# AbrahamSanders/realtime-codec-agent

Measured on AMD Instinct MI355X. Metric: batch-encode audio-hours/hour (+ xRT and p50 frame-step latency of 1 duplex stream in `duplex`), higher is better.
Workload: dtype f32; 1 GPU; batch MagiCodec-style encode, 16 kHz stereo, 0.1 s chunks / 2.0 s context, 256 windows per step (BASELINE configs[1]); codebook=131072x16

## Files before the change

realtime_codec_agent_amd/csrc/rca_codec.hip:

```cpp
#include <stdarg.h>

#include <algorithm>
#include <array>
#include <cmath>
#include <map>
#include <type_traits>

#include "rca_common.h"

namespace rca {
thread_local char g_err[512] = {0};
}
using namespace rca;

typedef float f32x16 __attribute__((ext_vector_type(16)));

#define RCA_LAT_MAX_FRAMES 64
#define RCA_LDS_BUDGET (152 * 1024)

typedef float f32x4 __attribute__((ext_vector_type(4)));

struct RowSrc {
    const float* base;
    int C;
    long chan_stride;
    long win_stride;
    int T;
    const long* row_off = nullptr;
    long span = 0;
    __device__ __forceinline__ long off(long b) const {
        return row_off ? row_off[b] : (b % C) * chan_stride + (b / C) * win_stride;
    }
};

__device__ __forceinline__ float lrelu(float v, float slope) { return v >= 0.0f ? v : v * slope; }

template <int KS>
__global__ __launch_bounds__(256) void conv_in_kernel(RowSrc src, const float* __restrict__ w,
                                                      const float* __restrict__ bias, float* __restrict__ y,
                                                      int B, int Cout, int Lout) {
    const long idx = (long)blockIdx.x * blockDim.x + threadIdx.x;
    if (idx >= (long)B * Lout) return;
    const int b = (int)(idx / Lout);
    const int t = (int)(idx - (long)b * Lout);
    const float* xr = src.base + src.off(b);
    constexpr int padL = KS / 2;
    float xv[KS];
#pragma unroll
    for (int kk = 0; kk < KS; ++kk) {
        const int i = t + kk - padL;
        xv[kk] = (i >= 0 && i < src.T) ? xr[i] : 0.0f;
    }
    float* yo = y + (long)b * Cout * Lout + t;
    for (int co = 0; co < Cout; ++co) {
        float acc = bias[co];
#pragma unroll
        for (int kk = 0; kk < KS; ++kk) {
            const int i = t + kk - padL;
            if (i >= 0 && i < src.T) acc = __builtin_fmaf(w[co * KS + kk], xv[kk], acc);
        }
        yo[(long)co * Lout] = acc;
    }
}

__global__ __launch_bounds__(256) void conv1d_chain_kernel(const float* __restrict__ x, const float* __restrict__ w,
                                                           const float* __restrict__ bias, float* __restrict__ y,
                                                           int B, int Cin, int Lin, int Cout, int Lout, int k, int s,
                                                           int pre, float slope, int clamp_out) {
    const long idx = (long)blockIdx.x * blockDim.x + threadIdx.x;
    if (idx >= (long)B * Cout * Lout) return;
    const int t = (int)(idx % Lout);
    const long r = idx / Lout;
    const int co = (int)(r % Cout);
    const int b = (int)(r / Cout);
    const int padL = (k - s + 1) / 2;
    const float* xb = x + (long)b * Cin * Lin;
    const float* wr = w + (long)co * Cin * k;
    float acc = bias[co];
    const int i0 = t * s - padL;
    for (int ci = 0; ci < Cin; ++ci) {
        const float* xr = xb + (long)ci * Lin;
        for (int kk = 0; kk < k; ++kk) {
            const int i = i0 + kk;
            if (i >= 0 && i < Lin) {
                float v = xr[i];
                if (pre) v = lrelu(v, slope);
                acc = __builtin_fmaf(wr[ci * k + kk], v, acc);
            }
        }
    }
    if (clamp_out) acc = acc > 1.0f ? 1.0f : (acc < -1.0f ? -1.0f : acc);
    y[idx] = acc;
}

__global__ __launch_bounds__(256) void convtr1d_chain_kernel(const float* __restrict__ x, const float* __restrict__ w,
                                                             const float* __restrict__ bias, float* __restrict__ y,
                                                             int B, int Cin, int Lin, int Cout, int k, int s, int pre,
                                                             float slope) {
    const int Lout = Lin * s;
    const long idx = (long)blockIdx.x * blockDim.x + threadIdx.x;
    if (idx >= (long)B * Cout * Lout) return;
    const int u = (int)(idx % Lout);
    const long r = idx / Lout;
    const int co = (int)(r % Cout);
    const int b = (int)(r / Cout);
    const int padL = (k - s + 1) / 2;
    const int kk0 = (u + padL) % s;
    const float* xb = x + (long)b * Cin * Lin;
    float acc = bias[co];
    for (int ci = 0; ci < Cin; ++ci) {
        const float* xr = xb + (long)ci * Lin;
        const float* wr = w + ((long)ci * Cout + co) * k;
        for (int kk = kk0; kk < k; kk += s) {
            const int t = (u + padL - kk) / s;
            if (t >= 0 && t < Lin) {
                float v = xr[t];
                if (pre) v = lrelu(v, slope);
                acc = __builtin_fmaf(wr[kk], v, acc);
            }
        }
    }
    y[idx] = acc;
}

typedef int rca_rsrc_t __attribute__((ext_vector_type(4)));
typedef float rca_f32x2_t __attribute__((ext_vector_type(2)));
__device__ float rca_buffer_load_f32(rca_rsrc_t rsrc, int voffset, int soffset, int aux) __asm("llvm.amdgcn.raw.buffer.load.f32");
__device__ rca_f32x2_t rca_buffer_load_f32x2(rca_rsrc_t rsrc, int voffset, int soffset, int aux) __asm("llvm.amdgcn.raw.buffer.load.v2f32");
typedef float rca_f32x4_t __attribute__((ext_vector_type(4)));
__device__ rca_f32x4_t rca_buffer_load_f32x4(rca_rsrc_t rsrc, int voffset, int soffset, int aux) __asm("llvm.amdgcn.raw.buffer.load.v4f32");
__device__ __forceinline__ rca_rsrc_t rca_make_rsrc(const void* base, int num_records) {
    const unsigned long a = (unsigned long)base;
    rca_rsrc_t r;
    r[0] = __builtin_amdgcn_readfirstlane((int)(unsigned)a);
    r[1] = __builtin_amdgcn_readfirstlane((int)((a >> 32) & 0xFFFF));
    r[2] = num_records;
    r[3] = 0x00020000;
    return r;
}

#ifdef RCA_CONV_TIMELINE
__device__ long* rca_prof_buf = nullptr;
#define RCA_TL_STAMP(v) const long v = tl_buf ? (long)wall_clock64() : 0
#define RCA_TL_ADD(acc, a, b) acc += (b) - (a)
#define RCA_TL_MIN(acc, a, b) acc = ((b) - (a)) < acc ? ((b) - (a)) : acc
#else
#define RCA_TL_STAMP(v)
#define RCA_TL_ADD(acc, a, b)
#define RCA_TL_MIN(acc, a, b)
#endif
template <int S>
struct ConvLds {
    static constexpr int want = (S == 8) ? 4 : (S == 4) ? 8 : (S == 2) ? 16 : (S == 5) ? 6 : 2;
    static constexpr int stride(int NT) {
        int u = NT + 2;
        while ((u % 32) != want % 32) ++u;
        return u;
    }
};

struct FuseIn {
    RowSrc src;
    const float* w_in;
    const float* b_in;
};
struct TrInfo {
    int s, padL, Lout, n_co;
};
template <int KS, int S, int TR>
struct ConvBOff {
    static constexpr int padL = (KS - S + 1) / 2;
    static constexpr int q_of(int kp, int half) {
        const int kl = 2 * kp + half, kk = kl % KS;
        const int d = TR ? -kk : kk - padL;
        return (d >= 0) ? d / S : -((-d + S - 1) / S);
    }
    static constexpr int off(int kp, int half, int U) {
        const int kl = 2 * kp + half, ci = kl / KS, kk = kl % KS;
        const int d = TR ? -kk : kk - padL;
        const int q = q_of(kp, half);
        return (ci * S + (d - q * S)) * U + 1 + q;
    }
    static constexpr int delta(int kp, int U) { return off(kp, 1, U) - off(kp, 0, U); }
    static constexpr int distinct(int k, int KPC, int U) {
        int found[4] = {0, 0, 0, 0};
        int n = 0;
        for (int kp = 0; kp < KPC; ++kp) {
            const int d = delta(kp, U);
            bool seen = false;
            for (int i = 0; i < n; ++i) seen = seen || found[i] == d;
            if (!seen && n < 4) found[n++] = d;
        }
        return found[k < n ? k : n - 1];
    }
    static constexpr int count(int KPC, int U) {
        int found[8] = {0, 0, 0, 0, 0, 0, 0, 0};
        int n = 0;
        for (int kp = 0; kp < KPC; ++kp) {
            const int d = delta(kp, U);
            bool seen = false;
            for (int i = 0; i < n; ++i) seen = seen || found[i] == d;
            if (!seen && n < 8) found[n++] = d;
        }
        return n;
    }
};

#ifndef RCA_CONV_WPB
#define RCA_CONV_WPB 1
#endif
#ifndef RCA_CONV_OCC
#define RCA_CONV_OCC 2
#endif
#ifndef RCA_CONV_PIPE
#define RCA_CONV_PIPE 1
#endif
#ifndef RCA_CONV_PRIO
#define RCA_CONV_PRIO 1
#endif
#ifndef RCA_CONV_ABUF
#define RCA_CONV_ABUF 1
#endif
#ifndef RCA_CONV_EPRIO
#define RCA_CONV_EPRIO 1
#endif
#ifdef RCA_ABL_NOBREAD
#define RCA_ABL_BREAD(x) (slope)
#else
#define RCA_ABL_BREAD(x) (x)
#endif
typedef __bf16 conv_bf16x8 __attribute__((ext_vector_type(8)));
typedef __bf16 conv_bf16x2 __attribute__((ext_vector_type(2)));
__device__ __forceinline__ unsigned conv_pack_bf16x2(float a, float b) {
    const conv_bf16x2 v = {(__bf16)a, (__bf16)b};
    return __builtin_bit_cast(unsigned, v);
}
template <int BF>
__device__ __forceinline__ void conv_split8(const float (&w)[8], uint4& hi, uint4& lo) {
    unsigned ph[4], pl[4];
#pragma unroll
    for (int j = 0; j < 4; ++j) {
        ph[j] = conv_pack_bf16x2(w[2 * j], w[2 * j + 1]);
        pl[j] = BF == 3 ? conv_pack_bf16x2(w[2 * j] - __uint_as_float(ph[j] << 16), w[2 * j + 1] - __uint_as_float(ph[j] & 0xffff0000u)) : 0u;
    }
    hi = make_uint4(ph[0], ph[1], ph[2], ph[3]);
    lo = make_uint4(pl[0], pl[1], pl[2], pl[3]);
}
template <int KS, int S, int CIC, int WM, int WN, int FUSE, int TR, int BF = 0, int FULLC = 0>
__global__ __launch_bounds__(64 * RCA_CONV_WPB, (((KS == 8 && CIC == 2) || (KS == 16 && CIC == 1)) && WM * WN < 8) ? 3 : RCA_CONV_OCC) void conv1d_mfma_kernel(const float* __restrict__ x, const float* __restrict__ wp,
                                                          const float* __restrict__ bias, float* __restrict__ y,
                                                          int Cin, int Lin, int Cout, int Lout, long Ncols, int nchunks,
                                                          int pre, float slope, FuseIn fin, TrInfo tr) {
    constexpr int MT = WM * 32;
    constexpr int NW = WN * 32;
    constexpr int U = ConvLds<S>::stride(NW);
    constexpr int KPC = CIC * KS / 2;
    constexpr int QPC = KPC / 4;
    constexpr int E = (NW + 2) * S;
    constexpr int PW = (S % 2 == 0 && !TR) ? 2 : 1;
    constexpr int RE = (E + 64 * PW - 1) / (64 * PW);
    constexpr int padL = (KS - S + 1) / 2;
    constexpr int BUF = CIC * S * U + 4;
    static_assert((CIC * KS) % 8 == 0, "chunk must hold whole weight quads");

    extern __shared__ __attribute__((aligned(16))) float xs_all[];
#ifdef RCA_CONV_TIMELINE
    long* const tl_buf = rca_prof_buf;
#endif
    RCA_TL_STAMP(tl0);

    const int lane = threadIdx.x & 63;
    const int half = lane >> 5;
    const int wave = __builtin_amdgcn_readfirstlane(threadIdx.x >> 6);
    float* xs = xs_all + wave * 2 * BUF;
    const int n_co_real = (Cout + MT - 1) / MT;
    const int n_co = TR ? n_co_real * tr.s : n_co_real;
    const long wg = blockIdx.x;
    const int xcd = (int)(wg & 7);
    const long seq = wg >> 3;
    const int co_tile_x = __builtin_amdgcn_readfirstlane((int)(seq % n_co));
    const int phase = TR ? co_tile_x / n_co_real : 0;
    const int co_tile = TR ? co_tile_x % n_co_real : co_tile_x;
    const long col_tile = (seq / n_co) * 8 + xcd;
// ... 296 lines not shown
#pragma unroll
            for (int wn = 0; wn < WN; ++wn) {
                float bv[8];
#pragma unroll
                for (int i = 0; i < 8; ++i) {
                    const int kp = g * 8 + i;
                    bv[i] = kp < KPC ? xb[b_off(kp < KPC ? kp : 0) + wn * 32] : 0.0f;
                    if (EDGE && kp < KPC && ((zmask[wn] >> kp) & 1u)) bv[i] = 0.0f;
                }
                conv_split8<BF>(bv, bh[wn], bl[wn]);
            }
#pragma unroll
            for (int wm = 0; wm < WM; ++wm) {
                float aw[8];
#pragma unroll
                for (int qq = 0; qq < 2; ++qq) {
                    const int q = 2 * g + qq;
                    const float4 q4 = q < QPC ? a[wm][q < QPC ? q : 0] : make_float4(0.0f, 0.0f, 0.0f, 0.0f);
                    aw[4 * qq + 0] = q4.x; aw[4 * qq + 1] = q4.y; aw[4 * qq + 2] = q4.z; aw[4 * qq + 3] = q4.w;
                }
                uint4 ah, al;
                conv_split8<BF>(aw, ah, al);
                const conv_bf16x8 ahv = __builtin_bit_cast(conv_bf16x8, ah), alv = __builtin_bit_cast(conv_bf16x8, al);
#pragma unroll
                for (int wn = 0; wn < WN; ++wn) {
                    const conv_bf16x8 bhv = __builtin_bit_cast(conv_bf16x8, bh[wn]);
                    acc[wm][wn] = __builtin_amdgcn_mfma_f32_32x32x16_bf16(ahv, bhv, acc[wm][wn], 0, 0, 0);
                    if (BF == 3) {
                        acc[wm][wn] = __builtin_amdgcn_mfma_f32_32x32x16_bf16(ahv, __builtin_bit_cast(conv_bf16x8, bl[wn]), acc[wm][wn], 0, 0, 0);
                        acc[wm][wn] = __builtin_amdgcn_mfma_f32_32x32x16_bf16(alv, bhv, acc[wm][wn], 0, 0, 0);
                    }
                }
#pragma unroll
                for (int qq = 0; qq < 2; ++qq) {
                    const int q = 2 * g + qq;
                    if (q < QPC) a[wm][q] = w_load(wm, cn, q);
                }
            }
        }
    };

    if (FUSE) stage_load(0);
    stage_write(0);
    __builtin_amdgcn_wave_barrier();
    if constexpr (PIPE) read_head(0);
    RCA_TL_STAMP(tl1);
#ifdef RCA_CONV_TIMELINE
    long tl_load = 1 << 30, tl_mfma = 0, tl_write = 0;
#endif
    const int lastc = nchunks - 1;
    auto chunk_loop = [&](auto edge_tag, auto act_tag) __attribute__((always_inline)) {
    for (int c = 0; c < nchunks; c += 2) {
        const int c1 = min(c + 1, lastc);
        RCA_TL_STAMP(ta);
        stage_load(c1);
        __builtin_amdgcn_sched_barrier(0);
        RCA_TL_STAMP(tb);
        __builtin_amdgcn_s_setprio(RCA_CONV_EPRIO);
        if constexpr (BF != 0) compute_b(0, c1, edge_tag);
        else if constexpr (PIPE) compute_p(0, c1, edge_tag);
        else compute_t(0, c1, edge_tag);
        __builtin_amdgcn_s_setprio(RCA_CONV_PRIO ? 3 : 2);
        __builtin_amdgcn_sched_barrier(0);
        RCA_TL_STAMP(tc);
        stage_write_t(1, act_tag);
        __builtin_amdgcn_wave_barrier();
        if constexpr (PIPE) {
            read_head(1);
            __builtin_amdgcn_sched_barrier(0);
        }
        RCA_TL_STAMP(td);
        RCA_TL_MIN(tl_load, tb, tc); RCA_TL_ADD(tl_mfma, tb, tc); RCA_TL_ADD(tl_write, tc, td);
        if (c + 1 >= nchunks) break;
        const int c2 = min(c + 2, lastc);
        stage_load(c2);
        __builtin_amdgcn_sched_barrier(0);
        __builtin_amdgcn_s_setprio(RCA_CONV_EPRIO);
        if constexpr (BF != 0) compute_b(1, c2, edge_tag);
        else if constexpr (PIPE) compute_p(1, c2, edge_tag);
        else compute_t(1, c2, edge_tag);
        __builtin_amdgcn_s_setprio(RCA_CONV_PRIO ? 3 : 2);
        __builtin_amdgcn_sched_barrier(0);
        stage_write_t(0, act_tag);
        __builtin_amdgcn_wave_barrier();
        if constexpr (PIPE) {
            read_head(0);
            __builtin_amdgcn_sched_barrier(0);
        }
    }
    };
    if (pre & 1) {
        if (edges) chunk_loop(std::true_type{}, std::true_type{});
        else chunk_loop(std::false_type{}, std::true_type{});
    } else {
        if (edges) chunk_loop(std::true_type{}, std::false_type{});
        else chunk_loop(std::false_type{}, std::false_type{});
    }

    if (RCA_CONV_EPRIO) __builtin_amdgcn_s_setprio(0);
    RCA_TL_STAMP(tl2);
    const long orow = TR ? tr.Lout : Lout;
    const bool full_rows = co0 + MT <= Cout;
    float* const yw = y + ((long)b_base * Cout + co0) * orow;
#pragma unroll
    for (int wn = 0; wn < WN; ++wn) {
        const int dn = 1 - lead + wn * 32 + (lane & 31);
        if (dn >= ncol_left) continue;
        int bb, t;
        rel_bt(dn, bb, t);
        int ocol = t;
        if (TR) {
            ocol = tr.s * t - tr.padL + phase;
            if (ocol < 0 || ocol >= (int)orow) continue;
        }
        const unsigned voff = ((unsigned)bb * (unsigned)(Cout * (int)orow) + (unsigned)ocol + (unsigned)(4 * half) * (unsigned)orow) * 4u;
        if (pre & 2) {
#pragma unroll
            for (int wm = 0; wm < WM; ++wm)
#pragma unroll
                for (int r = 0; r < 16; ++r) acc[wm][wn][r] = fmaxf(acc[wm][wn][r], acc[wm][wn][r] * slope);
        }
        if (full_rows) {
#pragma unroll
            for (int wm = 0; wm < WM; ++wm)
#pragma unroll
                for (int r = 0; r < 16; ++r) {
                    const int cu = wm * 32 + (r & 3) + 8 * (r >> 2);
                    char* const yr = reinterpret_cast<char*>(yw + (long)cu * orow);
                    *reinterpret_cast<float*>(yr + voff) = acc[wm][wn][r];
                }
        } else {
#pragma unroll
            for (int wm = 0; wm < WM; ++wm)
#pragma unroll
                for (int r = 0; r < 16; ++r) {
                    const int cu = wm * 32 + (r & 3) + 8 * (r >> 2);
                    char* const yr = reinterpret_cast<char*>(yw + (long)cu * orow);
                    if (co0 + cu + 4 * half < Cout) *reinterpret_cast<float*>(yr + voff) = acc[wm][wn][r];
                }
        }
    }
#ifdef RCA_CONV_TIMELINE
    if (tl_buf && lane == 0) {
        const long tl3 = (long)wall_clock64();
        const unsigned hw = __builtin_amdgcn_s_getreg((31 << 11) | (0 << 6) | 4);
        const unsigned xcc = __builtin_amdgcn_s_getreg((3 << 11) | (0 << 6) | 20);
        constexpr int region = KS == 4 ? 0 : KS == 8 ? 1 : KS == 10 ? 2 : KS == 16 ? 3 : KS == 3 ? 4 : 5;
        long* o = tl_buf + ((long)region * 65536 + ((blockIdx.x * RCA_CONV_WPB + wave) & 0xFFFF)) * 8;
        o[6] = tl_load | (tl_mfma << 32);
        o[7] = tl_write | ((long)nchunks << 32);
        o[0] = tl0; o[1] = tl1; o[2] = tl2; o[3] = tl3;
        o[4] = (long)hw | ((long)xcc << 32);
        o[5] = (long)KS | ((long)S << 8) | ((long)WM << 16) | ((long)wave << 24) | ((long)blockIdx.x << 32);
    }
#endif
}

template <int KS, int S, int CIC, int FUSE>
__global__ __launch_bounds__(512) void conv1d_ws_kernel(const float* __restrict__ x, const float* __restrict__ wp,
                                                        const float* __restrict__ bias, float* __restrict__ y,
                                                        int Cin, int Lin, int Cout, int Lout, long Ncols, int nchunks,
                                                        int pre, float slope, FuseIn fin) {
    constexpr int WM = 2, WN = 2;
    constexpr int MT = WM * 32, NW = WN * 32;
    constexpr int U = ConvLds<S>::stride(NW);
    constexpr int KPC = CIC * KS / 2;
    constexpr int QPC = KPC / 4;
    constexpr int E = (NW + 2) * S;
    constexpr int RE = (E + 63) / 64;
    constexpr int padL = (KS - S + 1) / 2;
    constexpr int BUF = CIC * S * U + 4;
    constexpr int WBUF = WM * QPC * 64 * 4;
    static_assert(KPC % 4 == 0 && KPC <= 64, "chunk shape");

    extern __shared__ __attribute__((aligned(16))) float lds[];
    float* aw_all = lds;
    float* xs_all = lds + 2 * WBUF;

    const int lane = threadIdx.x & 63;
    const int half = lane >> 5;
    const int wave = __builtin_amdgcn_readfirstlane(threadIdx.x >> 6);
    const bool producer = wave >= 4;
    const int cw = wave & 3;
    float* xs = xs_all + cw * 2 * BUF;

    const int n_co = (Cout + MT - 1) / MT;
    const long wg = blockIdx.x;
    const int xcd = (int)(wg & 7);
    const long seq = wg >> 3;
    const int co_tile = (int)(seq % n_co);
    const long col_tile = (seq / n_co) * 8 + xcd;
    const long n0 = (col_tile * 4 + cw) * NW;
    const int co0 = co_tile * MT;
    const bool active = n0 < Ncols;
    const long kquads = (long)nchunks * QPC;
    const int lastc = nchunks - 1;

    if (producer) {
        unsigned s_goff[RE];
        int s_loff[RE];
        bool s_ok[RE];
#pragma unroll
        for (int r = 0; r < RE; ++r) {
            const int e = lane + 64 * r;
            const int slot = e / S, p = e - slot * S;
            const long n = n0 - 1 + slot;
            s_ok[r] = active && e < E && n >= 0 && n < Ncols;
        s_loff[r] = e < E ? p * U + slot : -1;
            const long nn = s_ok[r] ? n : 0;
            const long b = nn / Lout;
            const int t = (int)(nn - b * Lout);
            s_goff[r] = s_ok[r] ? (unsigned)(b * Cin * (long)Lin + (long)t * S + p) : 0u;
        }
        float pc[FUSE ? RE : 1][7];
        if (FUSE) {
#pragma unroll
            for (int r = 0; r < RE; ++r) {
                const int e = lane + 64 * r;
                const int slot = e / S, p = e - slot * S;
                const long n = n0 - 1 + slot;
                const long nn = s_ok[r] ? n : 0;
                const long b = nn / Lout;
                const int i = (int)(nn - b * Lout) * S + p;
                const float* row = fin.src.base + fin.src.off(b);
#pragma unroll
                for (int kk = 0; kk < 7; ++kk) {
                    const int j = i + kk - 3;
                    pc[r][kk] = (s_ok[r] && j >= 0 && j < fin.src.T) ? row[j] : 0.0f;
                }
            }
        }
        const float act_slope = pre ? slope : 1.0f;
        constexpr int WITEMS = WM * QPC * 64;
        constexpr int WPER = (WITEMS + 255) / 256;
        const int ptid = threadIdx.x - 256;
        float sreg[CIC][RE];
        float4 wreg[WPER];
        auto issue_loads = [&](int c) {
#pragma unroll
            for (int i = 0; i < WPER; ++i) {
                const int it = ptid + 256 * i;
                const int itc = it < WITEMS ? it : 0;
                const int wm = itc / (QPC * 64), rem = itc - wm * (QPC * 64);
                const int cot = co_tile * WM + wm;
                wreg[i] = reinterpret_cast<const float4*>(wp)[((long)cot * kquads + (long)c * QPC) * 64 + rem];
            }
#pragma unroll
            for (int cl = 0; cl < CIC; ++cl) {
                const int ci = c * CIC + cl;
                if (FUSE) {
                    const int cc = ci < Cin ? ci : 0;
                    const float* wr = fin.w_in + cc * 7;
                    const float bi = fin.b_in[cc];
#pragma unroll
                    for (int r = 0; r < RE; ++r) {
                        float a = bi;
#pragma unroll
                        for (int kk = 0; kk < 7; ++kk) a = __builtin_fmaf(wr[kk], pc[r][kk], a);
                        sreg[cl][r] = a;
                    }
                } else {
                    const float* xc = x + (long)(ci < Cin ? ci : 0) * Lin;
#pragma unroll
                    for (int r = 0; r < RE; ++r) sreg[cl][r] = xc[s_goff[r]];
                }
            }
        };
        auto write_lds = [&](int c, int buf) {
            float4* aw = reinterpret_cast<float4*>(aw_all + buf * WBUF);
#pragma unroll
            for (int i = 0; i < WPER; ++i) {
                const int it = ptid + 256 * i;
                if (it < WITEMS) aw[it] = wreg[i];
            }
            float* dst = xs + buf * BUF;
#pragma unroll
            for (int cl = 0; cl < CIC; ++cl) {
                const bool cok = (c * CIC + cl) < Cin;
#pragma unroll
                for (int r = 0; r < RE; ++r) {
                    float v = (s_ok[r] && cok) ? sreg[cl][r] : 0.0f;
                    v = fmaxf(v, v * act_slope);
                    dst[s_loff[r] >= 0 ? cl * S * U + s_loff[r] : CIC * S * U] = v;
                }
            }
        };
        issue_loads(0);
        write_lds(0, 0);
        issue_loads(min(1, lastc));
        __syncthreads();
        for (int c = 0; c < nchunks; ++c) {
            const int c1 = min(c + 1, lastc);
            write_lds(c1, (c + 1) & 1);
            issue_loads(min(c + 2, lastc));
            __syncthreads();
        }
        return;
    }

    __builtin_amdgcn_s_setprio(3);
    int b_off[KPC];
    unsigned long long m_first = 0, m_last = 0;
#pragma unroll
    for (int kp = 0; kp < KPC; ++kp) {
        const int kl = 2 * kp + half;
        const int ci = kl / KS, kk = kl - ci * KS;
// ... 1084 lines not shown
    rca_codec* h = new rca_codec();
    h->cfg = *cfg;
    h->device = device;
    int rc = RCA_OK;
    auto bail = [&](int code) { rca_codec_destroy(h); return code; };
    if (hipStreamCreateWithFlags(&h->stream, hipStreamNonBlocking) != hipSuccess) return bail(fail(RCA_ERR_HIP, "stream create"));
    const int n = cfg->n_stages;
    h->hop = 1;
    for (int i = 0; i < n; ++i) h->hop *= cfg->strides[i];
    codec_receptive_field(*cfg, h->hop, &h->enc_left_frames, &h->dec_left_frames);

    auto add = [&](std::vector<ConvLayer>& v, const std::string& name, int cin, int cout, int k, int s, int pre, int tr,
                   bool pack) -> int {
        ConvLayer L;
        L.cin = cin; L.cout = cout; L.k = k; L.s = s; L.pre = pre; L.tr = tr;
        if ((rc = upload(ts, nt, name + ".weight", (long)cin * cout * k, &L.w)) != RCA_OK) return rc;
        if ((rc = upload(ts, nt, name + ".bias", cout, &L.b)) != RCA_OK) { v.push_back(L); return rc; }
        {
            const size_t nb = ((size_t)cout + 127) / 128 * 128 + 64;
            if (hipMalloc((void**)&L.bp, nb * 4) != hipSuccess || hipMemset(L.bp, 0, nb * 4) != hipSuccess ||
                hipMemcpy(L.bp, L.b, (size_t)cout * 4, hipMemcpyDeviceToDevice) != hipSuccess) {
                v.push_back(L);
                return fail(RCA_ERR_HIP, "bias pad alloc");
            }
        }
        if (pack && !tr && mfma_supported(k, s)) {
            const rca_tensor_t* t = find_tensor(ts, nt, name + ".weight");
            if ((rc = pack_weights((const float*)t->data, L)) != RCA_OK) { v.push_back(L); return rc; }
        }
        if (tr && k == 2 * s) {
            const rca_tensor_t* t = find_tensor(ts, nt, name + ".weight");
            if ((rc = pack_weights_tr((const float*)t->data, L)) != RCA_OK) { v.push_back(L); return rc; }
        }
        v.push_back(L);
        return RCA_OK;
    };
    if ((rc = add(h->enc, "enc.conv_in", 1, cfg->channels[0], cfg->k_in, 1, 0, 0, false)) != RCA_OK) return bail(rc);
    for (int i = 0; i < n; ++i) {
        const int s = cfg->strides[i];
        if ((rc = add(h->enc, "enc.down." + std::to_string(i), cfg->channels[i], cfg->channels[i + 1], 2 * s, s, 1, 0, true)) != RCA_OK)
            return bail(rc);
    }
    if ((rc = add(h->enc, "enc.conv_out", cfg->channels[n], cfg->latent_dim, cfg->k_latent, 1, 1, 0, true)) != RCA_OK) return bail(rc);
    if ((rc = add(h->dec, "dec.conv_in", cfg->codebook_dim, cfg->channels[n], cfg->k_latent, 1, 0, 0, true)) != RCA_OK) return bail(rc);
    for (int i = 0; i < n; ++i) {
        const int s = cfg->strides[n - 1 - i];
        if ((rc = add(h->dec, "dec.up." + std::to_string(i), cfg->channels[n - i], cfg->channels[n - 1 - i], 2 * s, s, 1, 1, false)) != RCA_OK)
            return bail(rc);
    }
    if ((rc = add(h->dec, "dec.conv_out", cfg->channels[0], 1, cfg->k_in, 1, 1, 0, false)) != RCA_OK) return bail(rc);

    const int J = cfg->codebook_dim, N = cfg->codebook_size, R = cfg->codebook_raw_dim, D = cfg->latent_dim;
    if ((rc = upload(ts, nt, "quantizer.in_proj.weight", (long)J * D, &h->q_in_w)) != RCA_OK) return bail(rc);
    if ((rc = upload(ts, nt, "quantizer.in_proj.bias", J, &h->q_in_b)) != RCA_OK) return bail(rc);
    float *raw = nullptr, *pw = nullptr, *pb = nullptr;
    auto free3 = [&]() { for (float* p : {raw, pw, pb}) if (p) (void)hipFree(p); };
    if ((rc = upload(ts, nt, "quantizer.codebook.weight", (long)N * R, &raw)) != RCA_OK) { free3(); return bail(rc); }
    if ((rc = upload(ts, nt, "quantizer.codebook_proj.weight", (long)J * R, &pw)) != RCA_OK) { free3(); return bail(rc); }
    if ((rc = upload(ts, nt, "quantizer.codebook_proj.bias", J, &pb)) != RCA_OK) { free3(); return bail(rc); }
    if (hipMalloc((void**)&h->cb, (size_t)N * J * 4) != hipSuccess || hipMalloc((void**)&h->hc, (size_t)N * 4) != hipSuccess ||
        hipMalloc((void**)&h->cbp, (size_t)N * J * 4) != hipSuccess || hipMalloc((void**)&h->err_flag, 4) != hipSuccess) {
        free3();
        return bail(fail(RCA_ERR_HIP, "codebook alloc"));
    }
    (void)hipMemsetAsync(h->err_flag, 0, 4, h->stream);
#ifdef RCA_CONV_TIMELINE
    if (getenv("RCA_CONV_TIMELINE_OUT")) {
        long* b = nullptr;
        (void)hipMalloc((void**)&b, (size_t)(6 << 16) * 8 * 8);
        (void)hipMemset(b, 0, (size_t)(6 << 16) * 8 * 8);
        (void)hipMemcpyToSymbol(HIP_SYMBOL(rca_prof_buf), &b, 8);
    }
#endif
    codebook_proj_kernel<<<cdiv((long)N * J, 256), 256, 0, h->stream>>>(raw, pw, pb, h->cb, N, R, J);
    codebook_norm_pack_kernel<<<cdiv(N, 256), 256, 0, h->stream>>>(h->cb, h->hc, h->cbp, N, J);
    hipError_t e = hipStreamSynchronize(h->stream);
    free3();
    if (e != hipSuccess) return bail(fail(RCA_ERR_HIP, "codebook init: %s", hipGetErrorString(e)));
    *out = h;
    return RCA_OK;
}

extern "C" int rca_codec_hop(const rca_codec_t* h, int32_t* hop) {
    if (!h || !hop) return fail(RCA_ERR_ARG, "null");
    *hop = h->hop;
    return RCA_OK;
}
extern "C" int rca_codec_num_frames(const rca_codec_t* h, int32_t T, int32_t* F) {
    if (!h || !F || T < 0) return fail(RCA_ERR_ARG, "bad argument");
    *F = (T + h->hop - 1) / h->hop;
    return RCA_OK;
}
extern "C" int rca_codec_set_variant(rca_codec_t* h, int32_t v) {
    if (!h || v < 0 || v > 2) return fail(RCA_ERR_ARG, "variant must be 0, 1 or 2");
    h->variant = v;
    return RCA_OK;
}
extern "C" int rca_codec_sync(rca_codec_t* h) {
    if (!h) return fail(RCA_ERR_ARG, "null");
    RCA_HIP(hipSetDevice(h->device));
    RCA_HIP(hipStreamSynchronize(h->stream));
    return RCA_OK;
}

template <int KS, int S, int CIC, int WM, int WN, int FUSE, int TR, int BF = 0>
static void launch_conv_cfg(const ConvLayer& L, const float* wp, int nchunks, const float* x, float* y, int Lin, int Lc, long Ncols,
                            float slope, const FuseIn& fin, const TrInfo& tr, hipStream_t st, int act) {
    constexpr int NT = RCA_CONV_WPB * WN * 32, MT = WM * 32;
    constexpr int lds = RCA_CONV_WPB * 2 * (CIC * S * ConvLds<S>::stride(WN * 32) + 4) * 4;
    static_assert(lds <= 65536, "LDS budget");
    const long col_tiles = (cdiv(Ncols, NT) + 7) / 8 * 8;
    dim3 grid((unsigned)(col_tiles * cdiv(L.cout, MT) * (TR ? tr.s : 1)));
    if constexpr (!FUSE && !TR && BF == 0) {
        if (L.cin % CIC == 0 && nchunks * CIC == L.cin) {
            conv1d_mfma_kernel<KS, S, CIC, WM, WN, 0, 0, 0, 1><<<grid, 64 * RCA_CONV_WPB, lds, st>>>(x, wp, L.bp, y, L.cin, Lin, L.cout, Lc, Ncols, nchunks, act, slope, fin, tr);
            return;
        }
    }
    conv1d_mfma_kernel<KS, S, CIC, WM, WN, FUSE, TR, BF><<<grid, 64 * RCA_CONV_WPB, lds, st>>>(x, wp, L.bp, y, L.cin, Lin, L.cout, Lc, Ncols, nchunks, act, slope, fin, tr);
}

template <int KS, int S, int CIC>
static int launch_conv_mfma(const ConvLayer& L, const float* x, float* y, int B, int Lin, int Lout, float slope, hipStream_t st,
                            const FuseIn* fuse = nullptr, int act = -1, int bf = 0) {
    if (act < 0) act = L.pre;
    const long Ncols = (long)B * Lout;
    if (bf) {
        const FuseIn none_b{};
        const TrInfo notr_b{};
        const bool big = (long)cdiv(Ncols, 64) * cdiv(L.cout, 64) >= 2048;
#define RCA_BF_LAUNCH(FU, BFM) do { \
            if (big) launch_conv_cfg<KS, S, CIC, 2, 2, FU, 0, BFM>(L, L.wp, L.nchunks, x, y, Lin, Lout, Ncols, slope, FU ? *fuse : none_b, notr_b, st, act); \
            else launch_conv_cfg<KS, S, CIC, 1, 1, FU, 0, BFM>(L, L.wp, L.nchunks, x, y, Lin, Lout, Ncols, slope, FU ? *fuse : none_b, notr_b, st, act); } while (0)
        if constexpr (KS == 4 || KS == 8 || KS == 16) {
            if (fuse) { if (bf == 3) RCA_BF_LAUNCH(1, 3); else RCA_BF_LAUNCH(1, 1); RCA_LAUNCH_CHECK(); return RCA_OK; }
        }
        if (fuse) return fail(RCA_ERR_ARG, "internal: fused first layer of this shape has no bf16 instantiation");
        if (bf == 3) RCA_BF_LAUNCH(0, 3); else RCA_BF_LAUNCH(0, 1);
#undef RCA_BF_LAUNCH
        RCA_LAUNCH_CHECK();
        return RCA_OK;
    }
    const long waves_big = (long)cdiv(Ncols, 64) * cdiv(L.cout, 64);
#ifdef RCA_CONV_FORCE_MID
    constexpr long BIG_MIN = 1L << 40, MID_MIN = 2048;
#else
    constexpr long BIG_MIN = 8192, MID_MIN = 2048;
#endif
    const FuseIn none{};
    const TrInfo notr{};
    if (fuse) {
        static const bool wide = []() { const char* e = getenv("RCA_FUSE_WIDE"); return !(e && e[0] == '0'); }();
        if constexpr (KS == 4 && S == 2) {
            if (wide && waves_big >= BIG_MIN && Lout >= 131 && L.cin % 2 == 0) {
                launch_conv_cfg<4, 2, 2, 2, 4, 1, 0>(L, L.wp, L.cin / 2, x, y, Lin, Lout, Ncols, slope, *fuse, notr, st, act);
                RCA_LAUNCH_CHECK();
                return RCA_OK;
            }
        }
        if (waves_big >= BIG_MIN) launch_conv_cfg<KS, S, CIC, 2, 2, 1, 0>(L, L.wp, L.nchunks, x, y, Lin, Lout, Ncols, slope, *fuse, notr, st, act);
        else launch_conv_cfg<KS, S, CIC, 1, 1, 1, 0>(L, L.wp, L.nchunks, x, y, Lin, Lout, Ncols, slope, *fuse, notr, st, act);
    } else {
        if (waves_big >= BIG_MIN) launch_conv_cfg<KS, S, CIC, 2, 2, 0, 0>(L, L.wp, L.nchunks, x, y, Lin, Lout, Ncols, slope, none, notr, st, act);
        else if (waves_big >= MID_MIN) launch_conv_cfg<KS, S, CIC, 1, 2, 0, 0>(L, L.wp, L.nchunks, x, y, Lin, Lout, Ncols, slope, none, notr, st, act);
        else if (KS == 3 && L.cout >= 64 && waves_big >= 1024) launch_conv_cfg<KS, S, CIC, (KS == 3 ? 2 : 1), 1, 0, 0>(L, L.wp, L.nchunks, x, y, Lin, Lout, Ncols, slope, none, notr, st, act);
        else launch_conv_cfg<KS, S, CIC, 1, 1, 0, 0>(L, L.wp, L.nchunks, x, y, Lin, Lout, Ncols, slope, none, notr, st, act);
    }
    RCA_LAUNCH_CHECK();
    return RCA_OK;
}

static int launch_convtr_mfma(const ConvLayer& L, const float* x, float* y, int B, int Lin, float slope, hipStream_t st) {
    const int Lc = Lin + 1;
    const long Ncols = (long)B * Lc;
    const FuseIn none{};
    const TrInfo tr{L.s, (L.k - L.s + 1) / 2, Lin * L.s, L.cout_pad / 32};
    const long waves_big = (long)cdiv(Ncols, 64) * cdiv(L.cout, 64) * L.s;
    if (L.cout > 32 && waves_big >= 2048) launch_conv_cfg<2, 1, 16, 2, 2, 0, 1>(L, L.wp_tr, L.nchunks_tr, x, y, Lin, Lc, Ncols, slope, none, tr, st, L.pre);
    else launch_conv_cfg<2, 1, 16, 1, 1, 0, 1>(L, L.wp_tr, L.nchunks_tr, x, y, Lin, Lc, Ncols, slope, none, tr, st, L.pre);
    RCA_LAUNCH_CHECK();
    return RCA_OK;
}

template <int KS, int S, int CIC, int FUSE>
static void launch_conv_ws(const ConvLayer& L, const float* x, float* y, int Lin, int Lout, long Ncols, float slope, const FuseIn& fin,
                           hipStream_t st) {
    constexpr int KPC = CIC * KS / 2, QPC = KPC / 4;
    constexpr int lds = (2 * (2 * QPC * 64 * 4) + 4 * 2 * (CIC * S * ConvLds<S>::stride(64) + 4)) * 4;
    static_assert(lds <= 160 * 1024, "LDS budget");
    auto kern = conv1d_ws_kernel<KS, S, CIC, FUSE>;
    static bool attr_done = false;
    if (!attr_done) { (void)hipFuncSetAttribute((const void*)kern, hipFuncAttributeMaxDynamicSharedMemorySize, lds); attr_done = true; }
    const long col_tiles = (cdiv(Ncols, 256) + 7) / 8 * 8;
    dim3 grid((unsigned)(col_tiles * cdiv(L.cout, 64)));
    kern<<<grid, 512, lds, st>>>(x, L.wp2, L.b, y, L.cin, Lin, L.cout, Lout, Ncols, L.nchunks2, L.pre, slope, fin);
}
static bool try_conv_ws(const ConvLayer& L, const float* x, float* y, int B, int Lin, int Lout, float slope, hipStream_t st, const FuseIn* fuse) {
    const long Ncols = (long)B * Lout;
    if (!L.wp2 || (long)cdiv(Ncols, 64) * cdiv(L.cout, 64) < 1024) return false;
    const FuseIn none{};
    if (L.k == 4 && L.s == 2) { if (fuse) launch_conv_ws<4, 2, 16, 1>(L, x, y, Lin, Lout, Ncols, slope, *fuse, st); else launch_conv_ws<4, 2, 16, 0>(L, x, y, Lin, Lout, Ncols, slope, none, st); }
    else if (L.k == 8 && L.s == 4 && !fuse) launch_conv_ws<8, 4, 8, 0>(L, x, y, Lin, Lout, Ncols, slope, none, st);
    else if (L.k == 16 && L.s == 8 && !fuse) launch_conv_ws<16, 8, 4, 0>(L, x, y, Lin, Lout, Ncols, slope, none, st);
    else if (L.k == 10 && L.s == 5 && !fuse) launch_conv_ws<10, 5, 8, 0>(L, x, y, Lin, Lout, Ncols, slope, none, st);
    else if (L.k == 3 && L.s == 1 && !fuse) launch_conv_ws<3, 1, 16, 0>(L, x, y, Lin, Lout, Ncols, slope, none, st);
    else return false;
    return true;
}

template <int K, int S, int NW>
static void launch_conv_lds(const ConvLayer& L, const float* x, long xbs, int Lvalid, float* y, int B, int Lin, int Lout, int NC, int W, int pre,
                            float slope, int clamp_out, hipStream_t st) {
    const size_t lds = ((size_t)W * (L.cin + 4) + (size_t)NW * L.cin * K) * 4;
    auto kern = conv1d_lds_kernel<K, S, NW>;
    static bool attr_done = false;
    if (!attr_done) { (void)hipFuncSetAttribute((const void*)kern, hipFuncAttributeMaxDynamicSharedMemorySize, RCA_LDS_BUDGET); attr_done = true; }
    dim3 grid(cdiv(Lout, NC), cdiv(L.cout, NW), B);
    kern<<<grid, 64 * NW, lds, st>>>(x, xbs, Lvalid, L.w, L.b, y, L.cin, Lin, L.cout, Lout, NC, W, slope, pre, clamp_out);
}
template <int S, int NW>
static void launch_convtr_lds(const ConvLayer& L, const float* x, float* y, int B, int Lin, int NC, int NTI, float slope, hipStream_t st) {
    const size_t lds = ((size_t)NTI * (L.cin + 4) + (size_t)NW * 2 * S * (L.cin + 4)) * 4;
    auto kern = convtr1d_lds_kernel<S, NW>;
    static bool attr_done = false;
    if (!attr_done) { (void)hipFuncSetAttribute((const void*)kern, hipFuncAttributeMaxDynamicSharedMemorySize, RCA_LDS_BUDGET); attr_done = true; }
    dim3 grid(cdiv((long)Lin * S, NC), cdiv(L.cout, NW), B);
    kern<<<grid, 64 * NW, lds, st>>>(x, L.w, L.w_lat, L.b, y, L.cin, Lin, L.cout, NC, NTI, slope, L.pre);
}
static bool try_conv_lds(rca_codec* h, const ConvLayer& L, const float* x, long xbs, int Lvalid, float* y, int B, int Lin, int clamp_out, hipStream_t st) {
    const float slope = h->cfg.leaky_slope;
    if (L.tr) {
        if (L.k != 2 * L.s) return false;
        const int Lout = Lin * L.s;
        const int NC = std::min(64, Lout);
        const int NTI = NC / L.s + 3;
        if (L.cin % 4 != 0) return false;
        auto fits = [&](int nw) { return ((size_t)NTI * (L.cin + 4) + (size_t)nw * L.k * (L.cin + 4)) * 4 <= RCA_LDS_BUDGET; };
#define RCA_TR(SS) if (L.s == SS) { if (fits(4)) launch_convtr_lds<SS, 4>(L, x, y, B, Lin, NC, NTI, slope, st); \
                                   else if (fits(2)) launch_convtr_lds<SS, 2>(L, x, y, B, Lin, NC, NTI, slope, st); \
                                   else if (fits(1)) launch_convtr_lds<SS, 1>(L, x, y, B, Lin, NC, NTI, slope, st); else return false; return true; }
        RCA_TR(2) RCA_TR(4) RCA_TR(5) RCA_TR(8)
#undef RCA_TR
        return false;
    }
    const int Lout = Lin / L.s;
    const int nw = L.cout >= 4 ? 4 : 1;
    int NC = std::min(64, Lout);
    auto W_of = [&](int nc) { return (nc * L.s + L.k - L.s + 3 + 3) & ~3; };
    auto lds_of = [&](int nc) { return ((size_t)W_of(nc) * (L.cin + 4) + (size_t)nw * L.cin * L.k) * 4; };
    while (NC > 1 && lds_of(NC) > RCA_LDS_BUDGET) NC = (NC + 1) / 2;
    if (lds_of(NC) > RCA_LDS_BUDGET || (L.cin >= 8 && 4 * L.k > 64)) return false;
    const int W = W_of(NC);
#define RCA_CV(KK, SS) if (L.k == KK && L.s == SS) { if (nw == 4) launch_conv_lds<KK, SS, 4>(L, x, xbs, Lvalid, y, B, Lin, Lout, NC, W, L.pre, slope, clamp_out, st); \
                                   else launch_conv_lds<KK, SS, 1>(L, x, xbs, Lvalid, y, B, Lin, Lout, NC, W, L.pre, slope, clamp_out, st); return true; }
    RCA_CV(4, 2) RCA_CV(8, 4) RCA_CV(10, 5) RCA_CV(16, 8) RCA_CV(3, 1) RCA_CV(7, 1)
#undef RCA_CV
    return false;
}

static bool mfma_conv_ok(const rca_codec* h, const ConvLayer& L, int B, int Lin, int clamp_out) {
    if (h->variant < 1 || L.tr || !L.wp || clamp_out || !mfma_supported(L.k, L.s)) return false;
    const int Lout = Lin / L.s;
    return (double)L.cin * Lin < 2.6e8 && (double)L.cout * Lin < 2.6e8 && (double)B * L.cin * Lin < 4.0e9 && (double)B * Lout < 2.0e9;
}

static int run_conv(rca_codec* h, const ConvLayer& L, const float* x, float* y, int B, int Lin, int clamp_out, hipStream_t st,
                    bool in_activated = false, bool want_post = false, bool* post_done = nullptr) {
    const float slope = h->cfg.leaky_slope;
    if (post_done) *post_done = false;
    if (in_activated && !(h->variant == 1 && !h->lat_mode && mfma_conv_ok(h, L, B, Lin, clamp_out)))
        return fail(RCA_ERR_ARG, "internal: activated input handed to a kernel without that mode");
    if (h->lat_mode && try_conv_lds(h, L, x, (long)L.cin * Lin, Lin, y, B, Lin, clamp_out, st)) {
        RCA_LAUNCH_CHECK();
        return RCA_OK;
    }
    const bool rows32 = (double)L.cin * Lin < 2.6e8 && (double)L.cout * Lin * (L.tr ? L.s : 1) < 2.6e8;
    if (L.tr && h->variant >= 1 && L.wp_tr && rows32 && (double)B * L.cin * Lin < 4.0e9 && (double)B * (Lin + 1) < 2.0e9) return launch_convtr_mfma(L, x, y, B, Lin, slope, st);
    if (L.tr) {
        const long total = (long)B * L.cout * Lin * L.s;
        convtr1d_chain_kernel<<<cdiv(total, 256), 256, 0, st>>>(x, L.w, L.b, y, B, L.cin, Lin, L.cout, L.k, L.s, L.pre, slope);
        RCA_LAUNCH_CHECK();
        return RCA_OK;
    }
    const int Lout = Lin / L.s;
    const double cflops = 2.0 * L.cin * L.k * L.cout * (double)B * Lout;
    const double cbytes = 4.0 * ((double)B * L.cin * Lin + (double)B * L.cout * Lout + (double)L.cin * L.k * L.cout);
    if (mfma_conv_ok(h, L, B, Lin, clamp_out)) {
        ProfScope ps(h, st, 0, cflops, cbytes);
        if (h->variant == 2 && try_conv_ws(L, x, y, B, Lin, Lout, slope, st, nullptr)) { RCA_LAUNCH_CHECK(); return RCA_OK; }
        const int act = ((L.pre && !in_activated) ? 1 : 0) | (want_post ? 2 : 0);
        if (post_done) *post_done = want_post;
        if (L.k == 4 && L.s == 2) return launch_conv_mfma<4, 2, 4>(L, x, y, B, Lin, Lout, slope, st, nullptr, act, h->mfma_mode);
        if (L.k == 8 && L.s == 4) return launch_conv_mfma<8, 4, RCA_CIC_K8>(L, x, y, B, Lin, Lout, slope, st, nullptr, act, h->mfma_mode);
        if (L.k == 10 && L.s == 5) return launch_conv_mfma<10, 5, 4>(L, x, y, B, Lin, Lout, slope, st, nullptr, act, h->mfma_mode);
        if (L.k == 16 && L.s == 8) return launch_conv_mfma<16, 8, RCA_CIC_K16>(L, x, y, B, Lin, Lout, slope, st, nullptr, act, h->mfma_mode);
        if (L.k == 3 && L.s == 1) return launch_conv_mfma<3, 1, RCA_CIC_K3>(L, x, y, B, Lin, Lout, slope, st, nullptr, act, h->mfma_mode);
    }
    if (in_activated) return fail(RCA_ERR_ARG, "internal: activated input handed to a kernel without that mode");
    const long total = (long)B * L.cout * Lout;
    ProfScope ps(h, st, 3, cflops, cbytes);
    conv1d_chain_kernel<<<cdiv(total, 256), 256, 0, st>>>(x, L.w, L.b, y, B, L.cin, Lin, L.cout, Lout, L.k, L.s, L.pre, slope, clamp_out);
    RCA_LAUNCH_CHECK();
    return RCA_OK;
}

static int pack_weights_bf16(const ConvLayer& L, Bf16Pack* out) {
// ... 717 lines not shown
```

Measured before the change: 3240 audio-hours/hour.

## Add dedicated MFMA kernel fusing input projection into first strided conv

```diff
diff --git a/realtime_codec_agent_amd/csrc/rca_codec.hip b/realtime_codec_agent_amd/csrc/rca_codec.hip
--- a/realtime_codec_agent_amd/csrc/rca_codec.hip
+++ b/realtime_codec_agent_amd/csrc/rca_codec.hip
@@ -129,6 +129,7 @@
 __device__ rca_f32x2_t rca_buffer_load_f32x2(rca_rsrc_t rsrc, int voffset, int soffset, int aux) __asm("llvm.amdgcn.raw.buffer.load.v2f32");
 typedef float rca_f32x4_t __attribute__((ext_vector_type(4)));
 __device__ rca_f32x4_t rca_buffer_load_f32x4(rca_rsrc_t rsrc, int voffset, int soffset, int aux) __asm("llvm.amdgcn.raw.buffer.load.v4f32");
+__device__ void rca_buffer_store_f32(float v, rca_rsrc_t rsrc, int voffset, int soffset, int aux) __asm("llvm.amdgcn.raw.buffer.store.f32");
 __device__ __forceinline__ rca_rsrc_t rca_make_rsrc(const void* base, int num_records) {
     const unsigned long a = (unsigned long)base;
     rca_rsrc_t r;
@@ -731,6 +732,220 @@
         o[0] = tl0; o[1] = tl1; o[2] = tl2; o[3] = tl3;
         o[4] = (long)hw | ((long)xcc << 32);
         o[5] = (long)KS | ((long)S << 8) | ((long)WM << 16) | ((long)wave << 24) | ((long)blockIdx.x << 32);
+    }
+#endif
+}
+
+template <int NWN, bool PRE>
+__global__ __launch_bounds__(64, 2) void conv_first_mfma_kernel(const float* __restrict__ wp, const float* __restrict__ bias,
+                                                               float* __restrict__ y, int Cout, int Lout, long Ncols, int post, float slope,
+                                                               FuseIn fin) {
+    constexpr int NW = NWN * 32;
+    constexpr int E = (NW + 2) * 2;
+    constexpr int NBLK = 2 * NWN + 1;
+    constexpr int RS = 136;
+    constexpr int ZERO = 128;
+    constexpr int CIN = 32, KQ = CIN / 2;
+    extern __shared__ __attribute__((aligned(16))) float ring[];
+#ifdef RCA_CONV_TIMELINE
+    long* const tl_buf = rca_prof_buf;
+#endif
+    RCA_TL_STAMP(tl0);
+    const int lane = threadIdx.x & 63;
+    const int half = lane >> 5, jl = lane & 31;
+    const int n_co = Cout / 64;
+    const long wg = blockIdx.x;
+    const int xcd = (int)(wg & 7);
+    const long seq = wg >> 3;
+    const int co_tile = __builtin_amdgcn_readfirstlane((int)(seq % n_co));
+    const long n0 = ((seq / n_co) * 8 + xcd) * NW;
+    const int co0 = co_tile * 64;
+    if (n0 >= Ncols) return;
+    const long n_base = n0 > 0 ? n0 - 1 : 0;
+    const int b_base = __builtin_amdgcn_readfirstlane((int)((unsigned)n_base / (unsigned)Lout));
+    const int t_base = (int)(n_base - (long)b_base * Lout);
+    const int lead = n0 > 0 ? 0 : 1;
+    const long left = Ncols - n_base;
+    const int ncol_left = left > NW + 2 ? NW + 2 : (int)left;
+    auto rel_bt = [&](int dn, int& bb, int& tt) {
+        int dt = dn + t_base;
+        bb = dt >= Lout ? 1 : 0;
+        tt = bb ? dt - Lout : dt;
+    };
+
+    const int ch_in = jl;
+    float a_in[4];
+#pragma unroll
+    for (int m = 0; m < 4; ++m) a_in[m] = (2 * m + half < 7) ? fin.w_in[ch_in * 7 + 2 * m + half] : -0.0f;
+    f32x16 b_in;
+#pragma unroll
+    for (int r = 0; r < 16; ++r) b_in[r] = fin.b_in[(r & 3) + 8 * (r >> 2) + 4 * half];
+    long o0, o1;
+    if (fin.src.row_off) {
+        const long nrows = (Ncols + Lout - 1) / Lout;
+        o0 = fin.src.row_off[b_base];
+        o1 = fin.src.row_off[b_base + 1 < nrows ? b_base + 1 : b_base];
+    } else {
+        const int C = fin.src.C;
+        const int c0 = b_base % C, w0 = b_base / C;
+        const int c1 = c0 + 1 == C ? 0 : c0 + 1, w1 = c0 + 1 == C ? w0 + 1 : w0;
+        o0 = (long)c0 * fin.src.chan_stride + (long)w0 * fin.src.win_stride;
+        o1 = (long)c1 * fin.src.chan_stride + (long)w1 * fin.src.win_stride;
+    }
+    const long om = o0 < o1 ? o0 : o1;
+    const rca_rsrc_t rs_pcm = rca_make_rsrc(fin.src.base + om, 0x7FFFFFFF);
+    const unsigned prow0 = (unsigned)(o0 - om), prow1 = (unsigned)(o1 - om);
+    constexpr unsigned OOB = 0x80000000u;
+    auto pcm_load = [&](int bk, float (&pb)[4]) __attribute__((always_inline)) {
+        const int e = 32 * bk + jl;
+        const int dn = (e >> 1) - lead;
+        const bool ok = e < E && dn >= 0 && dn < ncol_left;
+        int bb, t;
+        rel_bt(ok ? dn : 0, bb, t);
+        const int i = 2 * t + (e & 1) - 3 + half;
+        const unsigned ro = bb ? prow1 : prow0;
+#pragma unroll
+        for (int m = 0; m < 4; ++m) {
+            const int j = i + 2 * m;
+            const unsigned off = (ok && 2 * m + half < 7 && j >= 0 && j < fin.src.T) ? (ro + (unsigned)j) * 4u : OOB;
+            pb[m] = rca_buffer_load_f32(rs_pcm, (int)off, 0, 0);
+        }
+    };
+    auto cin_mfma = [&](int m, const float (&pb)[4], f32x16& d) __attribute__((always_inline)) {
+        d = __builtin_amdgcn_mfma_f32_32x32x2f32(a_in[m], pb[m], m == 0 ? b_in : d, 0, 0, 0);
+    };
+    const int w_lane = 4 * half * RS + jl;
+    auto cin_write = [&](int bk, f32x16& d, int r0, int r1) __attribute__((always_inline)) {
+#pragma unroll
+        for (int r = r0; r < r1; ++r) {
+            float v = d[r];
+            if (PRE) v = fmaxf(v, v * slope);
+            ring[w_lane + ((r & 3) + 8 * (r >> 2)) * RS + ((32 * bk) & 127)] = v;
+        }
+    };
+
+    if (lane < CIN) ring[lane * RS + ZERO] = 0.0f;
+    float pa[4], pb[4];
+    float4 a[2][KQ];
+    {
+        float p2[4];
+        pcm_load(0, pa);
+        pcm_load(1, pb);
+        pcm_load(2, p2);
+        __builtin_amdgcn_sched_barrier(0);
+        const rca_rsrc_t rs_w = rca_make_rsrc(reinterpret_cast<const float4*>(wp) + (long)co_tile * 2 * KQ * 64, 0x7FFFFFFF);
+#pragma unroll
+        for (int wm = 0; wm < 2; ++wm)
+#pragma unroll
+            for (int q = 0; q < KQ; ++q) {
+                const rca_f32x4_t v = rca_buffer_load_f32x4(rs_w, lane * 16, (wm * KQ + q) * 1024, 0);
+                a[wm][q] = make_float4(v[0], v[1], v[2], v[3]);
+            }
+        __builtin_amdgcn_sched_barrier(0);
+        f32x16 d0, d1;
+#pragma unroll
+        for (int m = 0; m < 4; ++m) { cin_mfma(m, pa, d0); cin_mfma(m, pb, d1); }
+        cin_write(0, d0, 0, 16);
+#pragma unroll
+        for (int m = 0; m < 4; ++m) cin_mfma(m, p2, d0);
+        cin_write(1, d1, 0, 16);
+        cin_write(2, d0, 0, 16);
+    }
+    if (NBLK > 3) pcm_load(3, pa);
+    if (NBLK > 4) pcm_load(4, pb);
+    __builtin_amdgcn_wave_barrier();
+    RCA_TL_STAMP(tl1);
+#ifdef RCA_CONV_TIMELINE
+    long tl_load = 1 << 30, tl_mfma = 0, tl_write = 0;
+#endif
+
+    const rca_rsrc_t rs_y = rca_make_rsrc(y + ((long)b_base * Cout + co0) * Lout, 0x7FFFFFFF);
+    __builtin_amdgcn_s_setprio(RCA_CONV_EPRIO);
+#pragma unroll
+    for (int wn = 0; wn < NWN; ++wn) {
+        RCA_TL_STAMP(ta);
+        const int j = 32 * wn + jl;
+        int bz, tz;
+        rel_bt(1 - lead + j, bz, tz);
+        const int ad0 = (half == 0 && tz == 0) ? ZERO : ((2 * j + 1 + half) & 127);
+        const int ad1 = (half == 1 && tz == Lout - 1) ? ZERO : ((2 * j + 3 + half) & 127);
+        f32x16 acc[2];
+#pragma unroll
+        for (int wm = 0; wm < 2; ++wm)
+#pragma unroll
+            for (int q = 0; q < 4; ++q) {
+                const f32x4 bq = *reinterpret_cast<const f32x4*>(bias + co0 + wm * 32 + 8 * q + 4 * half);
+#pragma unroll
+                for (int jj = 0; jj < 4; ++jj) acc[wm][4 * q + jj] = bq[jj];
+            }
+        const bool more = 2 * wn + 4 < NBLK;
+        f32x16 d;
+        float bcur[4], bnxt[4];
+        auto b_read = [&](int c, float (&bv)[4]) __attribute__((always_inline)) {
+#pragma unroll
+            for (int cl = 0; cl < 2; ++cl) {
+                bv[2 * cl] = ring[ad0 + (2 * c + cl) * RS];
+                bv[2 * cl + 1] = ring[ad1 + (2 * c + cl) * RS];
+            }
+        };
+        b_read(0, bcur);
+#pragma unroll
+        for (int c = 0; c < KQ; ++c) {
+            if (c + 1 < KQ) b_read(c + 1, bnxt);
+#pragma unroll
+            for (int kp = 0; kp < 4; ++kp) {
+#pragma unroll
+                for (int wm = 0; wm < 2; ++wm) {
+                    const float4 q4 = a[wm][c];
+                    const float av = kp == 0 ? q4.x : kp == 1 ? q4.y : kp == 2 ? q4.z : q4.w;
+                    acc[wm] = __builtin_amdgcn_mfma_f32_32x32x2f32(av, bcur[kp], acc[wm], 0, 0, 0);
+                }
+                if (c == 0 && 2 * wn + 3 < NBLK) cin_mfma(kp, pa, d);
+                if (c == 3 && more) cin_mfma(kp, pb, d);
+            }
+            if (c == 2 && 2 * wn + 3 < NBLK) cin_write(2 * wn + 3, d, 0, 16);
+            if (more && c >= 4 && (c & 3) == 3) cin_write(2 * wn + 4, d, 4 * (c >> 2) - 4, 4 * (c >> 2));
+            if (c == 1 && 2 * wn + 5 < NBLK) pcm_load(2 * wn + 5, pa);
+            if (c == 4 && 2 * wn + 6 < NBLK) pcm_load(2 * wn + 6, pb);
+            if (c + 1 < KQ) {
+#pragma unroll
+                for (int i = 0; i < 4; ++i) bcur[i] = bnxt[i];
+            }
+            __builtin_amdgcn_sched_barrier(0);
+        }
+        if (more) cin_write(2 * wn + 4, d, 12, 16);
+        __builtin_amdgcn_wave_barrier();
+        RCA_TL_STAMP(tb);
+        const int dn = 1 - lead + j;
+        int bb, t;
+        rel_bt(dn, bb, t);
+        const unsigned voff = dn < ncol_left ? ((unsigned)bb * (unsigned)(Cout * Lout) + (unsigned)t + (unsigned)(4 * half * Lout)) * 4u : OOB;
+        if (post) {
+#pragma unroll
+            for (int wm = 0; wm < 2; ++wm)
+#pragma unroll
+                for (int r = 0; r < 16; ++r) acc[wm][r] = fmaxf(acc[wm][r], acc[wm][r] * slope);
+        }
+#pragma unroll
+        for (int wm = 0; wm < 2; ++wm)
+#pragma unroll
+            for (int r = 0; r < 16; ++r) rca_buffer_store_f32(acc[wm][r], rs_y, (int)voff, (wm * 32 + (r & 3) + 8 * (r >> 2)) * Lout * 4, 0);
+        RCA_TL_STAMP(tc);
+        RCA_TL_MIN(tl_load, ta, tb); RCA_TL_ADD(tl_mfma, ta, tb); RCA_TL_ADD(tl_write, tb, tc);
+    }
+    if (RCA_CONV_EPRIO) __builtin_amdgcn_s_setprio(0);
+    RCA_TL_STAMP(tl2);
+#ifdef RCA_CONV_TIMELINE
+    if (tl_buf && lane == 0) {
+        const long tl3 = (long)wall_clock64();
+        const unsigned hw = __builtin_amdgcn_s_getreg((31 << 11) | (0 << 6) | 4);
+        const unsigned xcc = __builtin_amdgcn_s_getreg((3 << 11) | (0 << 6) | 20);
+        long* o = tl_buf + ((long)blockIdx.x & 0xFFFF) * 8;
+        o[6] = tl_load | (tl_mfma << 32);
+        o[7] = tl_write | ((long)(2 * NWN) << 32);
+        o[0] = tl0; o[1] = tl1; o[2] = tl2; o[3] = tl3;
+        o[4] = (long)hw | ((long)xcc << 32);
+        o[5] = 4L | (2L << 8) | (2L << 16) | ((long)blockIdx.x << 32);
     }
 #endif
 }
@@ -2121,6 +2336,17 @@
     if (fuse) {
         static const bool wide = []() { const char* e = getenv("RCA_FUSE_WIDE"); return !(e && e[0] == '0'); }();
         if constexpr (KS == 4 && S == 2) {
+            const char* mi = getenv("RCA_FUSE_MFMA_IN");
+            constexpr int NWN = 4;
+            if (!(mi && mi[0] == '0') && wide && waves_big >= BIG_MIN && Lout >= NWN * 32 + 3 && L.cin == 32 && L.cout % 64 == 0) {
+                const long col_tiles = (cdiv(Ncols, NWN * 32) + 7) / 8 * 8;
+                const dim3 grid((unsigned)(col_tiles * (L.cout / 64)));
+                constexpr int lds = 32 * 136 * 4;
+                if (act & 1) conv_first_mfma_kernel<NWN, true><<<grid, 64, lds, st>>>(L.wp, L.bp, y, L.cout, Lout, Ncols, act & 2, slope, *fuse);
+                else conv_first_mfma_kernel<NWN, false><<<grid, 64, lds, st>>>(L.wp, L.bp, y, L.cout, Lout, Ncols, act & 2, slope, *fuse);
+                RCA_LAUNCH_CHECK();
+                return RCA_OK;
+            }
             if (wide && waves_big >= BIG_MIN && Lout >= 131 && L.cin % 2 == 0) {
                 launch_conv_cfg<4, 2, 2, 2, 4, 1, 0>(L, L.wp, L.cin / 2, x, y, Lin, Lout, Ncols, slope, *fuse, notr, st, act);
                 RCA_LAUNCH_CHECK();
```

New measurement: 3319 audio-hours/hour, median of 6. 2.5% higher.
